# idra-lab/safe-mpc

Hardware: AMD Instinct MI355X
Metric: RTI-MPC instance-steps/s (batch=4096 per GPU, Z1 N=30) (higher is better)
Workload: dtype f64; 1 GPU; C1: Z1-class 6-DoF, N=30, 4096 instances/GPU, controller st (soft terminal NN row, MLP 12-256-256-256-1 fp32), EXT cost exact Hessian, 6 capsule pairs, Halton x0; batch_per_gpu=4096, batch_total=4096, horizon=30, controller=st, streams_per_gpu=3, qp_form=throughput, hip_graphs=False

## Files before the change

safe_mpc_amd/csrc/engine.hip:

```cpp
#include <hip/hip_runtime.h>

#include <cstdarg>
#include <cstdio>
#include <cstring>
#include <new>
#include <type_traits>
#include <vector>

#include "../../include/smpc.h"
#include "kernel_qp.hpp"
#include "kernel_qp_wg.hpp"
#include "kernel_build.hpp"
#include "kernels_callers.hpp"
#include "kernels_policy.hpp"
#include "kernels_mlp.hpp"
#include "kernels_nodes.hpp"
#include "kernels_sqp.hpp"
#include "kernels_guess.hpp"
#include "kernels_score.hpp"
#include "kernels_ik.hpp"
#include "kernels_rays.hpp"
#include "kernels_forecast.hpp"

using namespace smpc;
// ... 250 lines not shown
        if (!d) return nullptr;
        if (up && e == hipSuccess) e = hipMemcpyAsync(d, host, sizeof(T) * n, hipMemcpyHostToDevice, h->stream);
        if (down && host) back.push_back({(void*)host, d, sizeof(T) * n});
        return d;
    }
    template <class T> const T* in(const T* host, size_t n) { return view(host, n, true, false); }
    template <class T> T* out(T* host, size_t n) { return view(host, n, false, true); }
    template <class T> T* inout(T* host, size_t n) { return view(host, n, true, true); }

    template <class F> int place(F&& views) {
        views(*this);
        if (dev) return SMPC_OK;
        int rc;
        if ((rc = h->d_stage.reserve(h, "staging buffer", c.off))) return rc;
        c = Carve{h->d_stage.p};
        views(*this);
        if (e != hipSuccess) return fail(h, SMPC_EHIP, "staging copy failed: %s", hipGetErrorString(e));
        return SMPC_OK;
    }
    int finish() {
        if (dev) return SMPC_OK;
        for (const Back& b : back) HIPCHK(h, hipMemcpyAsync(b.host, b.dev, b.bytes, hipMemcpyDeviceToHost, h->stream));
        HIPCHK(h, hipStreamSynchronize(h->stream));
        return SMPC_OK;
    }
};

size_t ws_doubles_per_instance(smpc_handle* h, int N) {
    size_t per = 0;
    with_nq(h, [&](auto NQ) { per = QpLayout<NQ>(h->desc.n_rows).per_instance(N); return SMPC_OK; });
    return per;
}

int upload_bounds(smpc_handle* h, const double* lo, const double* hi) {
    const int nx = 2 * h->desc.nq;
    std::vector<double> l((size_t)(h->N + 1) * nx), u((size_t)(h->N + 1) * nx);
    for (int k = 0; k <= h->N; k++)
        for (int i = 0; i < nx; i++) {
            l[(size_t)k * nx + i] = lo ? lo[(size_t)k * nx + i] : (k == h->N ? h->desc.x_lo_e[i] : h->desc.x_lo[i]);
            u[(size_t)k * nx + i] = hi ? hi[(size_t)k * nx + i] : (k == h->N ? h->desc.x_hi_e[i] : h->desc.x_hi[i]);
        }
    int rc;
    if ((rc = h->d_lo.reserve(h, "stage bounds", l.size() * sizeof(double))) ||
        (rc = h->d_hi.reserve(h, "stage bounds", u.size() * sizeof(double))))
        return rc;
    HIPCHK(h, hipMemcpyAsync(h->d_lo.p, l.data(), l.size() * sizeof(double), hipMemcpyHostToDevice, h->stream));
    HIPCHK(h, hipMemcpyAsync(h->d_hi.p, u.data(), u.size() * sizeof(double), hipMemcpyHostToDevice, h->stream));
    HIPCHK(h, hipStreamSynchronize(h->stream));
    return SMPC_OK;
}

int ensure_mlp(smpc_handle* h, size_t M, int level = 2) {
    const size_t Mp = (M + 127) / 128 * 128, row = sizeof(float) * Mp, H = h->net->H;
    int rc;
    if ((rc = h->d_y.reserve(h, "network output", row))) return rc;
    for (int l = 0; level >= 1 && l + 1 < h->net->nlayers; l++)
        if ((rc = h->d_dg[l].reserve(h, "network activation derivatives", row * H))) return rc;
    if (level < 2) return SMPC_OK;
    if ((rc = h->d_S.reserve(h, "network features", row * MLP_KPAD)) || (rc = h->d_GS.reserve(h, "network gradients", row * MLP_NPAD)) ||
        (rc = h->d_dA.reserve(h, "network backward pass", row * H)) || (rc = h->d_dB.reserve(h, "network backward pass", row * H)))
        return rc;
    for (int l = 0; l + 1 < h->net->nlayers; l++)
        if ((rc = h->d_act[l].reserve(h, "network activations", row * H))) return rc;
    return SMPC_OK;
}

// ... 205 lines not shown
        return f > 0.0 && f <= 1.0 ? f : QP_CREW_DEFAULT;
    }();
    return v;
}
static int qp_crew_waves(const smpc_handle* h, int B) {
    const int pairs = (B + 1) / 2;
    if (h->qp_crew_waves > 0) return h->qp_crew_waves < pairs ? h->qp_crew_waves : pairs;
    const double f = h->qp_crew > 0.0 ? h->qp_crew : qp_crew_default();
    const int g = (int)ceil(f * pairs);
    return g < 1 ? 1 : (g > pairs ? pairs : g);
}

template <class F> int with_rows(const smpc_handle* h, F&& f) {
    switch (h->desc.n_rows) {
    case 6: return f(std::integral_constant<int, 6>{});
    case 4: return f(std::integral_constant<int, 4>{});
    default: return f(std::integral_constant<int, -1>{});
    }
}

int ensure_instance_bounds(smpc_handle* h, int B, bool zero) { return h->bounds.room(h, (size_t)2 * B * (h->N + 1) * 2 * h->desc.nq, zero); }
double* instance_hi(const smpc_handle* h) { return h->bounds.d.p ? h->bounds.d.p + h->bounds.d.cap / (2 * sizeof(double)) : nullptr; }

struct StageBounds {
    const double *lo, *hi;
    long stride;
};
StageBounds stage_bounds(const smpc_handle* h, int B) {
    if (const double* lo = h->bounds.for_batch(B)) return {lo, instance_hi(h), (long)(h->N + 1) * 2 * h->desc.nq};
    return {h->d_lo.p, h->d_hi.p, 0L};
}

template <int NQ>
int launch_stage_records(smpc_handle* h, int B, const double* x0, const double* xg, const double* ug, const double* p, bool timed) {
    int rc;
    if ((rc = launch_nn<NQ>(h, B, xg, p, h->d_nn.p, h->desc.nn_mode == SMPC_NN_TERMINAL ? 2 : 1))) return rc;
    if (timed) HIPCHK(h, hipEventRecord(h->ev_t[1], h->stream));
    const StageBounds bd = stage_bounds(h, B);
    const long nodes = (long)B * (h->N + 1);
    const dim3 grd((unsigned)((nodes + 64 / SB_G - 1) / (64 / SB_G))), blk(64);
    const double* nn = h->desc.nn_mode != SMPC_NN_NONE ? h->d_nn.p : nullptr;
    int32_t* const zero_cnt = h->desc.nn_mode == SMPC_NN_ALL ? h->d_nn_cnt : nullptr;
    with_rows(h, [&](auto MR) {
        return with_scene(h, B, [&](auto SCENE, auto sc) {
            return with_model(h, B, [&](auto MODEL, auto... md) {
                return with_row_bounds(h, B, [&](auto... rb) {
                    hipLaunchKernelGGL((k_stage_build<NQ, MR, SCENE, MODEL>), grd, blk, 0, h->stream, h->d_desc, B, h->N, x0, xg, ug, p, bd.lo,
                                       bd.hi, h->d_zl.p, nn, h->d_ws.p, bd.stride, h->d_active, zero_cnt, sc, md..., rb...);
                    return SMPC_OK;
                });
            });
        });
    });
    HIPCHK(h, hipGetLastError());
    if (timed) { HIPCHK(h, hipEventRecord(h->ev_t[2], h->stream)); HIPCHK(h, hipEventRecord(h->ev_t[4], h->stream)); }
    return SMPC_OK;
}

template <int NQ>
int launch_stage_records_per_node(smpc_handle* h, int B, const double* x0, const double* xg, const double* ug, const double* p) {
    int rc;
    if ((rc = launch_eval<NQ>(h, B, xg, ug, p, h->d_ev.p))) return rc;
    const StageBounds bd = stage_bounds(h, B);
    const int tiles = (int)ev_tiles((size_t)B * (h->N + 1));
    with_rows(h, [&](auto MR) {
        return with_row_bounds(h, B, [&](auto... rb) {
            hipLaunchKernelGGL((k_qp_setup<NQ, MR>), dim3(tiles), dim3(32 * EV_TILE), 0, h->stream, h->d_desc, B, h->N, x0, xg, ug, p, bd.lo,
                               bd.hi, h->d_zl.p, h->d_ev.p, h->d_ws.p, bd.stride, h->d_active, rb...);
            return SMPC_OK;
        });
    });
    HIPCHK(h, hipGetLastError());
    return SMPC_OK;
}

#ifndef QP_WG_FULL_BATCH
#define QP_WG_FULL_BATCH 256
#endif
#ifndef QP_WG_MAX_BATCH
#define QP_WG_MAX_BATCH 1024
#endif
static int qp_wg_mode() {
    static const int v = [] { const char* e = getenv("SMPC_QP_WG"); return e ? atoi(e) : -1; }();
    return v;
}
static int qp_wg_max_batch() {
    static const int v = [] { const char* e = getenv("SMPC_QP_WG_MAX_BATCH"); return e ? atoi(e) : QP_WG_MAX_BATCH; }();
    return v;
}
static int qp_wg_full_batch() {
    static const int v = [] { const char* e = getenv("SMPC_QP_WG_FULL_BATCH"); return e ? atoi(e) : QP_WG_FULL_BATCH; }();
    return v;
}
constexpr size_t QP_WG_LDS_LIMIT = 160 * 1024 - 512;

template <int NQ> int qp_wg_choice(const smpc_handle* h, int B) {
    const int mode = h->qp_mode >= -1 ? h->qp_mode : qp_wg_mode();
    if (mode == 0) return 0;
    if (mode < 0 && B > qp_wg_max_batch()) return 0;
    const auto fits = [&](int nhw) { return (size_t)WgLds<NQ>(h->N, h->desc.n_rows, nhw).total * sizeof(double) <= QP_WG_LDS_LIMIT; };
    if (B <= qp_wg_full_batch() && fits(8)) return 8;
    return fits(4) ? 4 : 0;
}

template <int NQ, int NHW>
int launch_qp_wg(smpc_handle* h, int B, const double* x0, const double* xg, const double* ug, double* xo, double* uo, int32_t* st,
                 int32_t* it) {
    if (h->d_hrec.cap < sizeof(double) * B * (h->N + 1) * HRecLayout<NQ>::SIZE)
        return fail(h, SMPC_ESTATE, "latency-form records not grown for %d instances", B);
    const size_t lds = (size_t)WgLds<NQ>(h->N, h->desc.n_rows, NHW).total * sizeof(double);
    return with_rows(h, [&](auto MR) {
        hipLaunchKernelGGL((k_qp_ipm_wg<NQ, MR, NHW>), dim3(B), dim3(32 * NHW), lds, h->stream, h->d_desc, B, h->N, x0, xg, ug, h->d_ws.p,
                           h->d_hrec.p, xo, uo, st, it, h->d_last_it.p, h->d_active, h->d_ord_hist.p);
        return SMPC_OK;
    });
}

template <int NQ, int NHW> int raise_qp_wg_lds_limit(smpc_handle* h) {
    if (h->wg_lds_raised[NHW == 8 ? 0 : 1]) return SMPC_OK;
    const int rc = with_rows(h, [&](auto MR) {
        HIPCHK(h, hipFuncSetAttribute(reinterpret_cast<const void*>(&k_qp_ipm_wg<NQ, MR, NHW>), hipFuncAttributeMaxDynamicSharedMemorySize,
                                      (int)QP_WG_LDS_LIMIT));
        return SMPC_OK;
    });
    h->wg_lds_raised[NHW == 8 ? 0 : 1] = rc == SMPC_OK;
    return rc;
}

template <int NQ> int ensure_qp_wg(smpc_handle* h, int B) {
    const int nhw = qp_wg_choice<NQ>(h, B);
    if (nhw == 0) return SMPC_OK;
    int rc;
    if ((rc = h->d_hrec.reserve(h, "latency-form records", sizeof(double) * B * (h->N + 1) * HRecLayout<NQ>::SIZE))) return rc;
    return nhw == 8 ? raise_qp_wg_lds_limit<NQ, 8>(h) : raise_qp_wg_lds_limit<NQ, 4>(h);
}

template <int NQ>
int launch_solve(smpc_handle* h, int B, const double* x0, const double* xg, const double* ug, const double* p,
                 double* xo, double* uo, int32_t* st, int32_t* it) {
    int rc;
    h->timing_now = false;
    if (h->timing) {
        h->timing_now = !capturing(h);
    }
    const bool timed = h->timing_now;
    if (timed) {
        h->ev_cur = (h->ev_cur + 1) % smpc_handle::EV_RING;
        h->ev_t = h->ev_sets[h->ev_cur];
        h->ev_complete[h->ev_cur] = false;
        h->timed_count++;
        HIPCHK(h, hipEventRecord(h->ev_t[0], h->stream));
    }
    if ((rc = launch_stage_records<NQ>(h, B, x0, xg, ug, p, timed))) return rc;
    const int wg_nhw = qp_wg_choice<NQ>(h, B);
    const bool wg = wg_nhw > 0;
    const int32_t* order = nullptr;
    if (h->order_B == B && B > 1 && !wg) {
        hipLaunchKernelGGL(k_order_by_iters, dim3((B + ORD_PER_BLOCK - 1) / ORD_PER_BLOCK), dim3(64), 0, h->stream, B, h->d_last_it.p,
                           h->d_order.p, h->d_ord_hist.p, h->d_ord_hist.p + 256, h->d_ord_hist.p + 512);
        order = h->d_order.p;
    } else {
        HIPCHK(h, hipMemsetAsync(h->d_ord_hist.p, 0, 520 * sizeof(int32_t), h->stream));
    }
    unsigned long long* wstat = nullptr;
    if (timed && h->timing == 1) {
        const unsigned long long init[4] = {0ull, ~0ull, 0ull, 0ull};
        HIPCHK(h, hipMemcpyAsync(h->d_wstat.p, init, sizeof(init), hipMemcpyHostToDevice, h->stream));
        wstat = h->d_wstat.p;
    }
    if (wg) {
        if ((rc = wg_nhw == 8 ? launch_qp_wg<NQ, 8>(h, B, x0, xg, ug, xo, uo, st, it) : launch_qp_wg<NQ, 4>(h, B, x0, xg, ug, xo, uo, st, it))) return rc;
    } else {
        const bool nt = qp_nt_mode() < 0 ? ws_doubles_per_instance(h, h->N) * sizeof(double) * (size_t)B >= qp_nt_threshold : qp_nt_mode() > 0;
        with_rows(h, [&](auto MR) {
            const auto launch = [&](auto NT) {
                hipLaunchKernelGGL((k_qp_ipm<NQ, MR, NT>), dim3(qp_crew_form<NQ, MR>() ? qp_crew_waves(h, B) : (B + 1) / 2), dim3(64), 0, h->stream, h->d_desc, B, h->N, x0, xg, ug,
                                   h->d_ws.p, xo, uo, st, it, order, h->d_last_it.p, wstat, h->d_active, h->d_ord_hist.p, h->d_ord_hist.p + 513);
                return SMPC_OK;
            };
            if constexpr (MR < 0) return launch(std::false_type{});
            else return nt ? launch(std::true_type{}) : launch(std::false_type{});
        });
    }
    h->order_B = B;
    HIPCHK(h, hipGetLastError());
    if (timed) {
        HIPCHK(h, hipEventRecord(h->ev_t[3], h->stream));
        h->ev_complete[h->ev_cur] = true;
        h->timed = 1;
    }
    return SMPC_OK;
}

struct ChkBlock { double *x_min, *x_max, *row_lb, *row_ub; size_t doubles; };
ChkBlock chk_block(double* base, int nq) {
    Carve m = dense(base);
    ChkBlock b{};
    b.x_min = m.take<double>(2 * nq);
    b.x_max = m.take<double>(2 * nq);
    b.row_lb = m.take<double>(SMPC_MAX_ROWS);
    b.row_ub = m.take<double>(SMPC_MAX_ROWS);
    b.doubles = m.off / sizeof(double);
    return b;
}
int upload_check_bounds(smpc_handle* h, const double* x_min, const double* x_max, const double* row_lb_chk,
                        const double* row_ub_chk) {
    const int nq = h->desc.nq, nr = h->desc.n_rows;
    std::vector<double> img(chk_block(nullptr, nq).doubles, 0.0);
    const ChkBlock b = chk_block(img.data(), nq);
    put(b.x_min, x_min, 2 * nq);
// ... 204 lines not shown
        h->d_active = nullptr;
        if (rc) { h->mlp_rows_hint = 0; return rc; }
        h->mlp_rows_hint = rows_test;
        hipLaunchKernelGGL(k_par_safe_list, grid(S * (N + 1)), blk, 0, s, (int)S, N, K, stepping, c.list, c.n_open, st->r, c.st,
                           h->d_nn_idx.p, h->d_nn_cnt);
        const ChkBlock cb = chk_block(h->chk.d.p, nq);
        const long M = S * (N + 1);
        rc = with_nq(h, [&](auto NQ) {
            hipLaunchKernelGGL((k_par_check_state<NQ>), grid(M), blk, 0, s, h->d_desc, (int)S, N, c.n_open, c.xo, cb.x_min, cb.x_max, par->tol_x,
                               cb.row_lb, cb.row_ub, c.st, c.ok, coll);
            HIPCHK(h, hipGetLastError());
            if (const int e = run_mlp<NQ>(h, (int)M, 3, 0, c.xo, false, rows_of_nodes(N + 1))) return e;
            hipLaunchKernelGGL((k_check_nn<NQ>), grid(M), blk, 0, s, h->d_desc, (int)M, c.xo, par->alpha, par->tol_safe, h->d_y.p, c.safe,
                               h->d_nn_idx.p, h->d_nn_cnt);
            HIPCHK(h, hipGetLastError());
            return SMPC_OK;
        });
        if (rc) { h->mlp_rows_hint = 0; return rc; }
    }
    h->mlp_rows_hint = 0;
    hipLaunchKernelGGL(k_par_select, grid(B), blk, 0, s, B, N, nq, stepping, d_ok, d_safe, c.pos, c.st, c.it, c.ok, c.safe, c.xo, c.uo,
                       st->x_temp, st->u_temp, st->status, st->qp_iter, st->x_guess, st->fails, st->current_step, st->r, st->x_viable,
                       d_acc, d_act, abort_out, any_abort, h->d_nn_cnt);
    hipLaunchKernelGGL(k_provide_control, grid((long)B * (nx + nq)), blk, 0, s, B, N, nq, d_acc, st->x_temp, st->u_temp, st->x_guess,
                       st->u_guess, u_out, stepping, d_act, u_other);
    HIPCHK(h, hipGetLastError());
    return SMPC_OK;
}

int ensure_batch(smpc_handle* h, int B, bool with_ev) {
    const size_t nodes = (size_t)B * (h->N + 1);
    const size_t nn_nodes = h->desc.nn_mode == SMPC_NN_NONE ? 0 : (h->desc.nn_mode == SMPC_NN_TERMINAL ? (size_t)B : nodes);
    int rc;
    if ((with_ev && (rc = h->d_ev.reserve(h, "linearisation records", sizeof(double) * ev_tiles(nodes) * EV_TILE * EV_D))) ||
        (rc = h->d_ws.reserve(h, "QP workspace", sizeof(double) * ws_doubles_per_instance(h, h->N) * B)) ||
        (rc = h->d_nn.reserve(h, "network rows", sizeof(double) * nn_nodes * (1 + 2 * h->desc.nq), true)) ||
        (rc = h->d_order.reserve(h, "dispatch order", sizeof(int32_t) * B)))
        return rc;
    const size_t had = h->d_last_it.cap;
    rc = h->d_last_it.reserve(h, "iteration counts", sizeof(int32_t) * B);
    if (h->d_last_it.cap != had) h->order_B = 0;
    if (rc || (rc = h->d_ord_hist.reserve(h, "iteration histogram", sizeof(int32_t) * 520, true))) return rc;
    return with_nq(h, [&](auto NQ) { return ensure_qp_wg<NQ>(h, B); });
}

struct SqpScratch {
    double *xs, *us, *dx, *du, *xt, *step, *m0t, *mt, *alpha, *m0, *Dd;
    int32_t *st, *it, *pos, *n_open;
    uint8_t *act, *settled, *trial;
    size_t bytes;
};
SqpScratch sqp_layout(char* base, int B, int N, int nq, bool full) {
    const size_t nX = (size_t)B * (N + 1) * 2 * nq, nU = (size_t)B * N * nq;
    Carve m{base};
    SqpScratch w{};
    w.xt = m.take<double>(nX);
    w.pos = m.take<int32_t>((size_t)B * (N + 1));
    if (full) {
        w.xs = m.take<double>(nX);
        w.us = m.take<double>(nU);
        w.dx = m.take<double>(nX);
        w.du = m.take<double>(nU);
        w.step = m.take<double>(B);
        w.m0t = m.take<double>((size_t)3 * B);
        w.mt = m.take<double>((size_t)3 * B);
        w.alpha = m.take<double>(B);
        w.m0 = m.take<double>(B);
        w.Dd = m.take<double>(B);
// ... 1586 lines not shown
        if (nc > ctx_cap) return fail(h, SMPC_EINVAL, "smpc_debug_scene_slots: the context holds %zu floats, room for %zu", nc, ctx_cap);
        HIPCHK(h, hipMemcpy(ctx_out, h->ctx.d.p, nc * sizeof(float), hipMemcpyDeviceToHost));
    }
    return SMPC_OK;
}

extern "C" int smpc_debug_qp_dispatch(smpc_handle* h, int32_t* out) {
    if (!h || !out) return SMPC_EINVAL;
    (void)hipSetDevice(h->device);
    if (!h->d_ord_hist.p) return fail(h, SMPC_ESTATE, "smpc_debug_qp_dispatch: no solve yet");
    HIPCHK(h, hipStreamSynchronize(h->stream));
    HIPCHK(h, hipMemcpy(out, h->d_ord_hist.p, 520 * sizeof(int32_t), hipMemcpyDeviceToHost));
    return SMPC_OK;
}

extern "C" int smpc_debug_stage_records(smpc_handle* h, int B, const double* x0, const double* xg, const double* ug, const double* p,
                                        int path, double* ws_out, int32_t* layout) {
    if (!h || B <= 0 || !x0 || !xg || !ug || !p || !ws_out || !layout) return SMPC_EINVAL;
    (void)hipSetDevice(h->device);
    int rc;
    if ((rc = guard_solve_slots(h, B, "smpc_debug_stage_records"))) return rc;
    if ((rc = ensure_batch(h, B))) return rc;
    const int N = h->N, nx = 2 * h->desc.nq, nu = h->desc.nq;
    Stage io{h, false};
    const double *dx0, *dxg, *dug, *dp;
    if ((rc = io.place([&](Stage& v) {
             dx0 = v.in(x0, (size_t)B * nx);
             dxg = v.in(xg, (size_t)B * (N + 1) * nx);
             dug = v.in(ug, (size_t)B * N * nu);
             dp = v.in(p, (size_t)B * (N + 1) * SMPC_NP);
         })))
        return rc;
    const size_t per = ws_doubles_per_instance(h, N);
    HIPCHK(h, hipMemsetAsync(h->d_ws.p, 0, per * (size_t)B * sizeof(double), h->stream));
    (void)&launch_stage_records<5>, (void)&launch_stage_records_per_node<5>;
    (void)&launch_stage_records<6>, (void)&launch_stage_records_per_node<6>;
    (void)&launch_stage_records<7>, (void)&launch_stage_records_per_node<7>;
    if ((rc = with_nq(h, [&](auto NQ) {
             return path == 1 ? launch_stage_records<NQ>(h, B, dx0, dxg, dug, dp, false) : launch_stage_records_per_node<NQ>(h, B, dx0, dxg, dug, dp);
         })))
        return rc;
    HIPCHK(h, hipMemcpyAsync(ws_out, h->d_ws.p, per * (size_t)B * sizeof(double), hipMemcpyDeviceToHost, h->stream));
    if ((rc = io.finish())) return rc;
    return with_nq(h, [&](auto NQ) {
        const QpLayout<NQ> Ly(h->desc.n_rows);
        const int v[24] = {Ly.stride, Ly.nIMG, Ly.oIMG, Ly.oSL, Ly.nF, Ly.oR0, Ly.oR1, Ly.oR2, Ly.oCZA, Ly.oCZN, Ly.oZ, Ly.oZN, Ly.NRT, Ly.nJ,
                           (int)per, 12, Ly.iTT, Ly.iGT, Ly.iGN, Ly.iB, Ly.iSC, Ly.iHQQ, Ly.iGZ, 0};
        for (int i = 0; i < 24; i++) layout[i] = v[i];
        return SMPC_OK;
    });
}

#ifdef QP_PROFILE
extern "C" int smpc_debug_qp_profile(unsigned long long* out16) {
    unsigned long long zero[16] = {0};
    if (hipMemcpyFromSymbol(out16, HIP_SYMBOL(smpc::g_qp_prof), sizeof(zero)) != hipSuccess) return -1;
    if (hipMemcpyToSymbol(HIP_SYMBOL(smpc::g_qp_prof), zero, sizeof(zero)) != hipSuccess) return -1;
    return 0;
}
extern "C" int smpc_debug_qp_wg_profile(unsigned long long* out16) {
    unsigned long long zero[16] = {0};
    if (hipMemcpyFromSymbol(out16, HIP_SYMBOL(smpc::g_wg_prof), sizeof(zero)) != hipSuccess) return -1;
    if (hipMemcpyToSymbol(HIP_SYMBOL(smpc::g_wg_prof), zero, sizeof(zero)) != hipSuccess) return -1;
    return 0;
}
#endif
```

safe_mpc_amd/csrc/kernel_build.hpp:

```cpp
#pragma once
#include "kernel_qp.hpp"
#include "rnea_deriv.hpp"

namespace smpc {

constexpr int SB_G = 8;
#ifndef SB_WAVES
#define SB_WAVES 2
#endif

template <int NQ, int MR_MAX> struct SbLds {
    static constexpr int NX = 2 * NQ;
    static constexpr int X_SC = 0, XA_END = 2 * NQ;
    static constexpr int X_SPC = 0, SPC_D = 24, XR_END = SPC_D * NQ;
    static constexpr int X_PT = 0, X_ZP = X_PT + 3 * SMPC_MAX_POINTS, XG_END = X_ZP + 9 * NQ;
    static constexpr int X_E = 0, X_Z0 = NX, X_GQ = X_Z0 + NX, XS_END = X_GQ + NQ;
    static constexpr int m1 = XA_END > XR_END ? XA_END : XR_END, m2 = XG_END > XS_END ? XG_END : XS_END;
    static constexpr int SIZE = qp_even_c(m1 > m2 ? m1 : m2);
};

template <int OFF> __device__ __forceinline__ double dpp_up(double x) {
    static_assert(OFF >= 1 && OFF <= 15, "row_shl:1..15");
    int lo = __double2loint(x), hi = __double2hiint(x);
    lo = __builtin_amdgcn_update_dpp(0, lo, 0x100 + OFF, 0xf, 0xf, true);
    hi = __builtin_amdgcn_update_dpp(0, hi, 0x100 + OFF, 0xf, 0xf, true);
    return __hiloint2double(hi, lo);
}

template <int CTRL> __device__ __forceinline__ double dpp_mov(double x) {
    int lo = __double2loint(x), hi = __double2hiint(x);
    lo = __builtin_amdgcn_update_dpp(0, lo, CTRL, 0xf, 0xf, true);
    hi = __builtin_amdgcn_update_dpp(0, hi, CTRL, 0xf, 0xf, true);
    return __hiloint2double(hi, lo);
}
__device__ __forceinline__ double grp_sum(double v) {
    v += dpp_mov<0xB1>(v);
    v += dpp_mov<0x4E>(v);
    v += dpp_mov<0x141>(v);
    return v;
}
__device__ __forceinline__ double grp_max(double v) {
    v = fmax(v, dpp_mov<0xB1>(v));
    v = fmax(v, dpp_mov<0x4E>(v));
    v = fmax(v, dpp_mov<0x141>(v));
    return v;
}

template <int NQ, int MRT, bool SCENE = false, bool MODEL = false, bool ROWB = false>
__device__ __forceinline__ void stage_build(const smpc_problem_desc* __restrict__ D, const QpLayout<NQ>& Ly, const int N, const int k,
                                            const bool valid, const int g, double* __restrict__ L, const double* __restrict__ x0b,
                                            const double* __restrict__ xk, const double* __restrict__ uk, const double* __restrict__ pk,
                                            const double* __restrict__ lo_k, const double* __restrict__ hi_k,
                                            const double* __restrict__ zl_st, const double* __restrict__ nnk, double* __restrict__ w,
                                            const double* __restrict__ geom_b = nullptr, const smpc_joint* __restrict__ Jb = nullptr,
                                            const double* __restrict__ rb_k = nullptr, const size_t rb_half = 0) {
    constexpr int NX = 2 * NQ, NU = NQ, NZ = 3 * NQ, NQP = QpLayout<NQ>::NQP, NZP = QpLayout<NQ>::NZP;
    constexpr int MR_MAX = MRT >= 0 ? MRT : SMPC_MAX_ROWS;
    constexpr int NSLOT = (MR_MAX + SB_G - 1) / SB_G;
    constexpr int NNL = SB_G - 1;
    static_assert(NQ < SB_G, "lane SB_G - 1 carries the network's row, lanes 0 .. NQ - 1 a joint each");
    static_assert(MR_MAX <= 2 * SB_G && 2 * NQ <= 2 * SB_G, "at most two collision rows and two box rows per lane");
    using LD = SbLds<NQ, MR_MAX>;
    const int MR = Ly.MR, MRP = Ly.MRP;
    const int rT0 = NX, rC0 = NX + NQ, rNN = NX + NQ + MR;
    const bool last = (k == N);
    const bool jl = g < NQ;
    const int gj = jl ? g : NQ - 1;
    double* const sX = L;
    const double dt = D->dt, cB = 0.5 * dt * dt;

    double qd[NQ], qdd[NQ];
#pragma unroll
    for (int i = 0; i < NQ; i++) {
        qd[i] = xk[NQ + i];
        qdd[i] = last ? 0.0 : uk[i];
    }
    {
        double s, c;
        sincos(xk[gj], &s, &c);
        if (jl) { sX[LD::X_SC + 2 * g] = s; sX[LD::X_SC + 2 * g + 1] = c; }
    }
    lds_fence();

// ... 308 lines not shown
    }
    double* const sE = sX + LD::X_E;
    double* const sZ0 = sX + LD::X_Z0;
    double* const sGQ = sX + LD::X_GQ;
    for (int i = g; i < NX; i += SB_G) sZ0[i] = k == 0 ? x0b[i] - xk[i] : 0.0;
    if (jl) sGQ[g] = gz_q;
    lds_fence();
    double bmax = 0.0;
    auto defect = [&](int i) -> double {
        if (last) return 0.0;
        const double* xn = xk + NX;
        const int ii = i < NQ ? i : i - NQ;
        const double ukk = uk[ii];
        return i < NQ ? xk[ii] + dt * xk[NQ + ii] + cB * ukk - xn[ii] : xk[NQ + ii] + dt * ukk - xn[NQ + ii];
    };
    for (int i = g; i < NX; i += SB_G) {
        const double bb = defect(i);
        bmax = fmax(bmax, fabs(bb));
        if (valid) *(w + Ly.oIMG + Ly.iB + i) = bb;
    }
    bmax = grp_max(bmax);
    const double bflag = bmax > 0.0 ? 1.0 : 0.0;
    auto gz_u = [&](int c) -> double { return (reach && !last) ? cs * 2.0 * D->R * uk[c] : 0.0; };
    for (int hz = g; hz < NZP; hz += SB_G) {
        if (hz >= NU && hz < NU + NQ) continue;
        if (valid) *(w + Ly.oIMG + Ly.iGZ + hz) = hz < NU ? gz_u(hz) : 0.0;
    }
    if (jl && valid) *(w + Ly.oIMG + Ly.iGZ + NU + g) = gz_q;
    if (g < 4 && valid) {
        const double huu = (reach && !last ? cs * 2.0 * D->R : 0.0) + lm;
        *(w + Ly.oIMG + Ly.iSC + g) = g == 0 ? huu : (g == 1 ? lm : (g == 2 ? wsoft : bflag));
        *(w + Ly.oSL + g) = g == 0 ? wsoft : (g == 1 ? bflag : 0.0);
    }
    if (valid) *(w + Ly.oWC + g) = 0.0;

    double r0_loc = 0.0, mu_acc = 0.0, inf0 = 0.0;
    int cnt = 0;
    auto init_row = [&](bool present, int r, double lo, double hi, double cz, double cn, bool soft) -> double {
        double tl = 1.0, ll = 0.0, tu = 1.0, lu = 0.0;
        if (present) {
            const double thr = soft ? QP_THR : QP_THR_HARD * (cn > 0.0 ? cn : 1.0);
            if (lo > -QP_ABSENT) {
                const double s0 = soft ? QP_THR : 0.0;
                const double slack = cz + s0 - lo;
                tl = fmax(slack, thr);
                ll = D->qp_mu0 / tl;
                if (soft) ll = fmin(ll, 0.5 * wsoft);
                r0_loc = fmax(r0_loc, fabs(slack - tl));
                cnt += soft ? 2 : 1;
                mu_acc += ll * tl;
                if (soft) { mu_acc += (wsoft - ll) * s0; tu = s0; }
            }
            if (hi < QP_ABSENT) {
                const double slack = hi - cz;
                tu = fmax(slack, thr);
                lu = D->qp_mu0 / tu;
                r0_loc = fmax(r0_loc, fabs(slack - tu));
                cnt += 1;
                mu_acc += lu * tu;
            }
            if (valid) {
                reinterpret_cast<dbl2*>(w + Ly.oR0)[r] = dbl2{lo, hi};
                reinterpret_cast<dbl2*>(w + Ly.oR1)[r] = dbl2{tl, tu};
                reinterpret_cast<dbl2*>(w + Ly.oR2)[r] = dbl2{ll, lu};
            }
        }
        return -(ll - lu);
// ... 35 lines not shown
        } else {
            if (k >= 1 && fabs(row.lb) < SMPC_INF) lo = row.lb - growv[sl];
            if (k >= 1 && fabs(row.ub) < SMPC_INF) hi = row.ub - growv[sl];
        }
#pragma unroll
        for (int j = 0; j < NQ; j++) cn = fmax(cn, fabs(grow[sl][j]));
        if (k == 0) {
#pragma unroll
            for (int j = 0; j < NQ; j++) cz = fma(grow[sl][j], sZ0[j], cz);
        }
        eC[sl] = init_row(have, rC0 + r, lo, hi, cz, cn, false);
        if (!have) eC[sl] = 0.0;
        if (have && k == 0 && D->rows_at_node0) {
            const double v = growv[sl] + cz;
            if constexpr (ROWB) {
                if ((fabs(lb) < SMPC_INF && v < lb - D->qp_tol) || (fabs(ub) < SMPC_INF && v > ub + D->qp_tol)) inf0 = 1.0;
            } else {
                if ((fabs(row.lb) < SMPC_INF && v < row.lb - D->qp_tol) || (fabs(row.ub) < SMPC_INF && v > row.ub + D->qp_tol)) inf0 = 1.0;
            }
        }
    }
    double eN = 0.0;
    {
        const bool mine = g == NNL;
        double lo = -QP_ABSENT, cn = 0.0;
        if (nn_on && mine) {
            lo = 0.0 - nnk[0];
            for (int i = 0; i < NX; i++) cn = fmax(cn, fabs(nnk[1 + i]));
        }
        eN = init_row(mine, rNN, lo, QP_ABSENT, 0.0, cn, wsoft >= 0.0);
        if (!mine) eN = 0.0;
    }
    for (int r = g; r < 32; r += SB_G)
        if (valid) { *(w + Ly.oCZA + r) = 0.0; *(w + Ly.oCZN + r) = 0.0; }
    for (int hz = g; hz < NZ; hz += SB_G) {
        const double z0 = hz >= NU ? sZ0[hz - NU] : 0.0;
        if (valid) { *(w + Ly.oZ + hz) = z0; *(w + Ly.oZN + hz) = z0; }
    }
    lds_fence();
    {
        double pc[NZ];
#pragma unroll
        for (int c = 0; c < NZ; c++) pc[c] = rowT[c] * eT;
#pragma unroll
        for (int sl = 0; sl < NSLOT; sl++)
#pragma unroll
            for (int j = 0; j < NQ; j++) pc[NU + j] = fma(grow[sl][j], eC[sl], pc[NU + j]);
        if (nn_on && g == NNL) {
#pragma unroll
            for (int i = 0; i < NX; i++) pc[NU + i] = fma(nnk[1 + i], eN, pc[NU + i]);
        }
#pragma unroll
        for (int c = 0; c < NZ; c++) {
            const double sc = grp_sum(pc[c]);
            const bool skip = (k == 0 && c >= NU) || (last && c < NU);
            const double gz = c < NU ? gz_u(c) : (c < NU + NQ ? sGQ[c - NU] : 0.0);
            const double a = gz + sc + (c >= NU ? sE[c - NU] : 0.0);
            r0_loc = fmax(r0_loc, skip ? 0.0 : fabs(a));
        }
    }
    if (!last) {
        for (int i = g; i < NX; i += SB_G) {
            double ax = 0.0;
            if (k == 0) ax = i < NQ ? sZ0[i] + dt * sZ0[NQ + i] : sZ0[i];
            r0_loc = fmax(r0_loc, fabs(ax + defect(i)));
        }
    }
    const double R0 = grp_max(r0_loc), musum = grp_sum(mu_acc), cntsum = grp_sum((double)cnt), infs = grp_max(inf0);
    if (g < 4 && valid) w[Ly.oPART + g] = g == 0 ? R0 : (g == 1 ? musum : (g == 2 ? cntsum : infs));

    if (valid) {
        double* img = w + Ly.oIMG;
        if (g < NQP) {
#pragma unroll
            for (int c = 0; c < NZ; c++) *(img + Ly.iTT + c * NQP + g) = rowT[c];
        }
#pragma unroll
        for (int sl = 0; sl < NSLOT; sl++) {
            const int r = g + SB_G * sl;
            if (r < MRP) {
#pragma unroll
                for (int j = 0; j < NQ; j++) *(img + Ly.iGT + j * MRP + r) = grow[sl][j];
            }
        }
        if (g == NNL)
            for (int i = 0; i < NX; i++) *(img + Ly.iGN + i) = nn_on ? nnk[1 + i] : 0.0;
    }
    lds_fence();
}

template <int NQ, int MRT, bool SCENE = false, bool MODEL = false, class... MJ>
__global__ __launch_bounds__(64) __attribute__((amdgpu_waves_per_eu(SB_WAVES, SB_WAVES))) void k_stage_build(const smpc_problem_desc* __restrict__ D, int B, int N, const double* __restrict__ x0,
                                                    const double* __restrict__ xg, const double* __restrict__ ug, const double* __restrict__ pp,
                                                    const double* __restrict__ lo_st, const double* __restrict__ hi_st,
                                                    const double* __restrict__ zl_st, const double* __restrict__ nn, double* __restrict__ ws_all,
                                                    long bnd_stride, const uint8_t* __restrict__ active, int32_t* __restrict__ zero_cnt,
                                                    const SceneArg<SCENE> sc = {}, const MJ* __restrict__... md) {
    static_assert(ModelRowArg<MODEL, MJ...>, "md: the table of smpc_joint records when MODEL is set, then the row-bounds table or nothing");
    constexpr bool ROWB = RowBounds<MJ...>;
    constexpr int NX = 2 * NQ, NU = NQ;
    constexpr int MR_MAX = MRT >= 0 ? MRT : SMPC_MAX_ROWS;
    using LD = SbLds<NQ, MR_MAX>;
    if (zero_cnt && blockIdx.x == 0 && threadIdx.x == 0) *zero_cnt = 0;
    constexpr int NODES = 64 / SB_G;
    __shared__ __attribute__((aligned(16))) double smem[NODES * LD::SIZE];
    const int g = threadIdx.x & (SB_G - 1), grp = threadIdx.x / SB_G;
    const long total = (long)B * (N + 1);
    long t = (long)blockIdx.x * NODES + grp;
    bool valid = t < total;
    if (!valid) t = total - 1;
    const long b = t / (N + 1);
    const int k = (int)(t - b * (N + 1));
    if (active && !active[b]) valid = false;
    const QpLayout<NQ> Ly(MRT >= 0 ? MRT : D->n_rows);
    double* w = ws_all + (size_t)b * Ly.per_instance(N) + (size_t)k * Ly.stride;
    const double* xk = xg + ((size_t)b * (N + 1) + k) * NX;
    const double* uk = ug + ((size_t)b * N + (k < N ? k : N - 1)) * NU;
    const double* pk = pp + ((size_t)b * (N + 1) + k) * SMPC_NP;
    const size_t bo = (size_t)b * bnd_stride + (size_t)k * NX;
    const double* geom_b = nullptr;
    if constexpr (SCENE) geom_b = scene_block(sc, b, scene_time(sc) + k, Ly.MR);
    const smpc_joint* Jb = nullptr;
    if constexpr (MODEL) Jb = model_joints<NQ>(D, b, md...);
    const double* rb_k = nullptr;
    size_t rb_half = 0;
    if constexpr (ROWB) {
        rb_k = row_bounds_table(md...) + ((size_t)b * (N + 1) + k) * Ly.MR;
        rb_half = (size_t)B * (N + 1) * Ly.MR;
    }
    stage_build<NQ, MRT, SCENE, MODEL, ROWB>(D, Ly, N, k, valid, g, smem + grp * LD::SIZE, x0 + (size_t)b * NX, xk, uk, pk, lo_st + bo, hi_st + bo, zl_st,
                                nn ? nn + (D->nn_mode == SMPC_NN_TERMINAL ? (size_t)b : (size_t)b * (N + 1) + k) * (1 + NX) : nullptr, w,
                                geom_b, Jb, rb_k, rb_half);
}

}
```

safe_mpc_amd/csrc/kernel_qp.hpp:

```cpp
#pragma once
#include <type_traits>

#include "device_model.hpp"

namespace smpc {

constexpr double QP_THR = 1e-1;
constexpr double QP_THR_HARD = 3e-2;
constexpr double QP_FTB = 0.995;
constexpr double QP_ALPHA_MIN = 1e-12;
constexpr double QP_ABSENT = 1e300;

constexpr int qp_even_c(int n) { return (n + 1) & ~1; }
constexpr int qp_al8(int n) { return (n + 7) & ~7; }

template <int NQ> struct QpLayout {
    static constexpr int NX = 2 * NQ, NU = NQ, NZ = 3 * NQ;
    static constexpr int NZP = qp_even_c(NZ), NQP = qp_even_c(NQ), WS2 = qp_even_c(NX + 1);
    static constexpr int LC0 = WS2;
    static constexpr int KS = qp_even_c(LC0 + NQ);
    static constexpr int WR = NX + 1, LOFF = NQ * WR, NWP = qp_even_c(LOFF + NQ * (NQ + 1) / 2);
    __host__ __device__ static constexpr int w_coff(int j) { return LOFF + j * NQ - j * (j - 1) / 2; }
    int MR, MRP, NRC, NRT;
    int iTT, iGT, iGN, iHQQ, iGZ, iB, iSC, nIMG;
    int nJ;
    int nF;
    int oIMG, oW, oSL, oPART, oWC, oR0, oR1, oR2, oCZA, oCZN;
    int oZ, oZN, oA12;
    int stride;
    __host__ __device__ explicit QpLayout(int n_rows) {
        MR = n_rows;
        MRP = qp_even_c(MR);
        NRC = NQ + MR + 1;
        NRT = NX + NRC;
        int i = 0;
        iTT = i; i += NZ * NQP;
        iGT = i; i += NQ * MRP;
        iGN = i; i += NX;
        nJ = i;
        iB = i; i += NX;
        iSC = i; i += 4;
        nF = i;
        iHQQ = i; i += qp_even_c(NQ * NQ);
        iGZ = i; i += NZP;
        nIMG = i;
        int o = 0;
        oIMG = o; o += qp_al8(nIMG);
        oW = o; o += qp_al8(NWP);
        oSL = o; o += 16;
        oPART = oSL + 4;
        oWC = oSL + 8;
        oR0 = o; o += qp_al8(NRT * 2);
        oR1 = o; o += qp_al8(NRT * 2);
        oR2 = o; o += qp_al8(NRT * 2);
        oCZA = o; o += 32;
        oCZN = o; o += 32;
        oZ = o; o += qp_al8(NZ);
        oZN = o; o += qp_al8(NZ);
        oA12 = o; o += qp_al8(2 * NZ);
        static_assert(NQ <= 8, "the corrector's w shares a 16-double block with the stage scalars");
        stride = (o + 15) & ~15;
    }
    __host__ __device__ size_t per_instance(int N) const { return (size_t)stride * (N + 1); }
};

typedef double dbl2 __attribute__((ext_vector_type(2)));


__device__ __forceinline__ void lds_fence() {
    __builtin_amdgcn_fence(__ATOMIC_ACQ_REL, "wavefront", "local");
    __builtin_amdgcn_wave_barrier();
}

__device__ __forceinline__ void hold(double& a, double& b, double& c, double& d) { asm volatile("" : "+v"(a), "+v"(b), "+v"(c), "+v"(d)); }
template <int H> __device__ __forceinline__ void hold_rows2(dbl2 (&a)[H], dbl2 (&b)[H], double (&s)[5]) {
    static_assert(H == 3 || H == 4, "NQP / 2 of the built sizes");
    if constexpr (H == 3)
        asm volatile("" : "+v"(a[0]), "+v"(a[1]), "+v"(a[2]), "+v"(b[0]), "+v"(b[1]), "+v"(b[2]), "+v"(s[0]), "+v"(s[1]), "+v"(s[2]),
                          "+v"(s[3]), "+v"(s[4]));
    else
        asm volatile("" : "+v"(a[0]), "+v"(a[1]), "+v"(a[2]), "+v"(a[3]), "+v"(b[0]), "+v"(b[1]), "+v"(b[2]), "+v"(b[3]), "+v"(s[0]),
                          "+v"(s[1]), "+v"(s[2]), "+v"(s[3]), "+v"(s[4]));
}
template <int H> __device__ __forceinline__ void hold_rows4(dbl2 (&a)[H], dbl2 (&b)[H], dbl2 (&c)[H], dbl2 (&d)[H], double (&s)[9]) {
    static_assert(H == 3 || H == 4, "NQP / 2 of the built sizes");
    if constexpr (H == 3)
        asm volatile("" : "+v"(a[0]), "+v"(a[1]), "+v"(a[2]), "+v"(b[0]), "+v"(b[1]), "+v"(b[2]), "+v"(c[0]), "+v"(c[1]), "+v"(c[2]),
// ... 302 lines not shown
                cn = 0.0;
                for (int c = 0; c < NZ; c++) {
                    const double cv = sC[(r - NX) * NZP + c];
                    cz = fma(cv, sZ0[c], cz);
                    cn = fmax(cn, fabs(cv));
                }
            }
            const bool soft = (r == rNN) && wsoft >= 0.0;
            const double thr = soft ? QP_THR : QP_THR_HARD * (cn > 0.0 ? cn : 1.0);
            if (sLO[r] > -QP_ABSENT) {
                const double s0 = soft ? QP_THR : 0.0;
                const double slack = cz + s0 - sLO[r];
                tl = fmax(slack, thr);
                ll = D->qp_mu0 / tl;
                if (soft) ll = fmin(ll, 0.5 * wsoft);
                r0_loc = fmax(r0_loc, fabs(slack - tl));
                cnt += soft ? 2 : 1;
                mu_acc += ll * tl;
                if (soft) { mu_acc += (wsoft - ll) * s0; tu = s0; }
            }
            if (sHI[r] < QP_ABSENT) {
                const double slack = sHI[r] - cz;
                tu = fmax(slack, thr);
                lu = D->qp_mu0 / tu;
                r0_loc = fmax(r0_loc, fabs(slack - tu));
                cnt += 1;
                mu_acc += lu * tu;
            }
        }
        if (r < NRT) {
            reinterpret_cast<dbl2*>(w + Ly.oR1)[r] = dbl2{tl, tu};
            reinterpret_cast<dbl2*>(w + Ly.oR2)[r] = dbl2{ll, lu};
        }
        *(w + Ly.oCZA + hl) = 0.0;
        *(w + Ly.oCZN + hl) = 0.0;
        sE[r] = -(ll - lu);
    }
    if (hl < 4) *(w + Ly.oSL + hl) = hl == 0 ? wsoft : (hl == 1 ? bflag : 0.0);
    if (hl < 8) *(w + Ly.oWC + hl) = 0.0;
    if (hl < NZ) { *(w + Ly.oZ + hl) = sZ0[hl]; *(w + Ly.oZN + hl) = sZ0[hl]; }
    lds_fence();
    if (hl < NZ && !(k == 0 && hl >= NU) && !(last && hl < NU)) {
        double a = sGZ[hl];
        for (int r = 0; r < NRC; r++) a = fma(sC[r * NZP + hl], sE[NX + r], a);
        if (hl >= NU) a += sE[hl - NU];
        r0_loc = fmax(r0_loc, fabs(a));
    }
    if (!last && hl < NX) {
        double ax = 0.0;
        if (k == 0) ax = hl < NQ ? sZ0[NU + hl] + dt * sZ0[NU + NQ + hl] : sZ0[NU + hl];
        r0_loc = fmax(r0_loc, fabs(ax + sB[hl]));
    }
    double inf0 = 0.0;
    if (k == 0 && D->rows_at_node0 && hl >= rC0 && hl < rNN) {
        const smpc_row& row = D->rows[hl - rC0];
        double v = e.row_val[hl - rC0];
        for (int c = 0; c < NZ; c++) v = fma(sC[(hl - NX) * NZP + c], sZ0[c], v);
        if constexpr (RowBounds<RB...>) {
            const RowLbUb own = row_bounds_at(row_bounds_table(rb...), B, N, MR, b, k, hl - rC0);
            if ((fabs(own.lb) < SMPC_INF && v < own.lb - D->qp_tol) || (fabs(own.ub) < SMPC_INF && v > own.ub + D->qp_tol)) inf0 = 1.0;
        } else {
            if ((fabs(row.lb) < SMPC_INF && v < row.lb - D->qp_tol) || (fabs(row.ub) < SMPC_INF && v > row.ub + D->qp_tol)) inf0 = 1.0;
        }
    }
    const double R0 = half_max(r0_loc), musum = half_sum(mu_acc), cntsum = half_sum((double)cnt), infs = half_max(inf0);
    if (hl < 4) w[Ly.oPART + hl] = hl == 0 ? R0 : (hl == 1 ? musum : (hl == 2 ? cntsum : infs));
}

#ifndef QP_WAVES_PER_EU
#define QP_WAVES_PER_EU 2
#endif

template <int NQ, int MRT> constexpr bool qp_crew_form() { return !(NQ == 6 && MRT < 0); }
// ... 230 lines not shown
    const double inv_m = 1.0 / (double)m_comp;
    QPT(13);

    double rho_lin = 1.0, alpha = 0.0, sigmu = 0.0, corr_w = 1.0;
    bool pending = false;
    int it = 0, st_code = 2;
    const double tol = D->qp_tol;
    const double tol_r = D->qp_tol_res > 0.0 ? D->qp_tol_res : D->qp_tol;
    const int max_iter = D->qp_max_iter;
    const int stall_max = D->qp_stall_iters;
    int stall = 0;
    bool broke = false;
    double *Pc = sIMG + O_PA, *Pn = sIMG + O_PB2;
    double *pvc = sIMG + O_PVA, *pvn = sIMG + O_PVB;
    lds_fence();

    for (it = 0; it < max_iter; it++) {
        if (mu <= tol && rho_lin * R0 <= tol_r) { st_code = 0; break; }

        double mu_new = 0.0;
        {
            dbl2 img[IMG_PF];
            QpRow rs;
            dbl2 slb;
            double zc, znc, czar, cznr;
            auto load_b1 = [&](int k) {
                const double* w = stage_ptr(k);
                const dbl2* s2 = reinterpret_cast<const dbl2*>(w + Ly.oIMG);
#pragma unroll
                for (int j = 0; j < IMG_PF; j++) img[j] = ldnt(s2 + min(hl + 32 * j, img_n2 - 1));
                const dbl2 r0 = ldnt(reinterpret_cast<const dbl2*>(w + Ly.oR0) + hr), r1 = ldnt(reinterpret_cast<const dbl2*>(w + Ly.oR1) + hr),
                           r2 = ldnt(reinterpret_cast<const dbl2*>(w + Ly.oR2) + hr);
                rs.lo = r0.x; rs.hi = r0.y; rs.tl = r1.x; rs.tu = r1.y; rs.ll = r2.x; rs.lu = r2.y;
                czar = *(w + Ly.oCZA + hr);
                cznr = *(w + Ly.oCZN + hr);
                slb = *reinterpret_cast<const dbl2*>(w + Ly.oSL);
                zc = *(w + Ly.oZ + hz);
                znc = *(w + Ly.oZN + hz);
            };
            auto stage_b1 = [&](int k, auto last_tag) {
                constexpr bool last = decltype(last_tag)::value;
                asm volatile("; QPMARK B1_BEGIN");
                double* w = stage_ptr(k);
                {
                    dbl2* d2 = reinterpret_cast<dbl2*>(sIMG);
#pragma unroll
                    for (int j = 0; j < IMG_PF; j++) d2[min(hl + 32 * j, img_n2 - 1)] = img[j];
                }
                const double wsoft = slb.x;
                const bool bflag = !last && slb.y != 0.0;
                {
                    const bool soft = soft_lane && wsoft >= 0.0;
                    double rr_ = 0.0, s1_ = 0.0, s2_ = 0.0;
                    const QpDir rd = qp_row_dir<false>(rs, soft, wsoft, cznr, sigmu, corr_w, czar, &rr_, &s1_, &s2_, nullptr, nullptr);
                    rs.tl += alpha * rd.dtl; rs.ll += alpha * rd.dll;
                    rs.tu += alpha * rd.dtu; rs.lu += alpha * rd.dlu;
                    stnt_b1(dbl2{rs.tl, rs.tu}, reinterpret_cast<dbl2*>(w + Ly.oR1) + hr);
                    stnt_b1(dbl2{rs.ll, rs.lu}, reinterpret_cast<dbl2*>(w + Ly.oR2) + hr);
                    double Dr;
                    sE[hr] = qp_row_coeff(rs, soft, wsoft, 0.0, 0.0, 0.0, &Dr);
                    sD[hr] = Dr;
                    mu_new += row_live ? qp_row_comp(rs, soft, wsoft) : 0.0;
                }
                zc += alpha * (znc - zc);
                *(w + Ly.oZ + hz) = zc;
                lds_fence();
                QPT(0);
                load_b1(k > 0 ? k - 1 : 0);
                {
                    double a = bflag ? pdot(Pc + hl_x * NX, sB, NX / 2) : 0.0;
                    if constexpr (last && PASS_TAB) asm volatile("" : "+v"(a));
// ... 622 lines not shown
        __builtin_amdgcn_fence(__ATOMIC_RELEASE, "workgroup");

        double rr_max, S1c, S2c;
        sweep_f(std::true_type{}, &rr_max, &S1c, &S2c);
        __builtin_amdgcn_fence(__ATOMIC_RELEASE, "workgroup");
        const double a_max = rr_max > 0.0 ? 1.0 / rr_max : 1e300;
        const double tau_k = a_max >= 0.99 ? fmin(0.9999, fmax(QP_FTB, 1.0 - mu)) : QP_FTB;
        alpha = fmin(1.0, tau_k * a_max);
        if (!(alpha == alpha)) { st_code = 4; break; }
        if (alpha < QP_ALPHA_MIN) { st_code = 3; break; }
        pending = true;
        rho_lin *= (1.0 - alpha);
        const double mu_before = mu;
        mu = (mu * (double)m_comp + alpha * S1c + alpha * alpha * S2c) * inv_m;
        if (!(mu == mu)) { st_code = 4; pending = false; break; }
        {
            const bool stalled = alpha < 0.5 && !(mu < 0.5 * mu_before);
            stall = stalled ? stall + 0x10001 : (stall & ~0xffff);
        }
        if (stall_max > 0 && ((stall & 0xffff) >= stall_max || (stall >> 16) >= stall_max + (stall_max + 5) / 6) &&
            !(mu <= tol && rho_lin * R0 <= tol_r)) { st_code = 5; it++; break; }
    }
    if (it == max_iter && st_code == 2 && mu <= tol && rho_lin * R0 <= tol_r) st_code = 0;

    bool bad = false;
    const double a_fin = pending ? alpha : 0.0;
    constexpr int EP_CH = 8;
    for (int k0 = 0; k0 <= N; k0 += EP_CH) {
        double zz[EP_CH], zzn[EP_CH], bb[EP_CH];
#pragma unroll
        for (int j = 0; j < EP_CH; j++) {
            const int k = k0 + j <= N ? k0 + j : N;
            const double* w = ws + (size_t)k * Ly.stride;
            zz[j] = *(w + Ly.oZ + hz);
            zzn[j] = *(w + Ly.oZN + hz);
            const int ku = k < N ? k : N - 1;
            bb[j] = hl < NU ? ub0[(size_t)ku * NU + hl_u] : xb0[(size_t)k * NX + hl_px];
        }
#pragma unroll
        for (int j = 0; j < EP_CH; j++) {
            const int k = k0 + j;
            const double v = pending ? bb[j] + zz[j] + a_fin * (zzn[j] - zz[j]) : bb[j] + zz[j];
            if (k <= N) {
                if (hl < NU) {
                    if (k < N) { u_out[((size_t)b * N + k) * NU + hl] = v; bad |= !(v == v); }
                } else if (hl < NZ) {
                    x_out[((size_t)b * (N + 1) + k) * NX + hl - NU] = v;
                    bad |= !(v == v);
                }
            }
        }
    }
    const bool any_bad = half_max(bad ? 1.0 : 0.0) > 0.0;
#ifdef QP_PROFILE
    QPT(12);
    if (hl == 0) {
        for (int i = 0; i < 14; i++) atomicAdd(&g_qp_prof[i], tacc[i]);
        atomicAdd(&g_qp_prof[14], 1ull);
        atomicAdd(&g_qp_prof[15], (unsigned long long)it);
    }
#endif
    if (wstat && hl == 0) {
        const unsigned long long t_end = __builtin_amdgcn_s_memrealtime(), t_begin = s_tbegin[half];
        atomicAdd(&wstat[0], t_end - t_begin);
        atomicMin(&wstat[1], t_begin);
        atomicMax(&wstat[2], t_end);
        atomicAdd(&wstat[3], 1ull);
// ... 66 lines not shown
```

Measured before the change: 1.147 million instance-steps/s.

## Skip per-stage zeroing of iterate slots via shared zero header in workspace

Adds a zeroed header block ahead of the QP workspace. On the first IPM iteration, stages k>0 read their initial CZA/CZN/Z values from that shared header instead of their own slots, so the stage-build and setup kernels no longer write zeros and initial iterates for every stage (only k==0, or all stages when the workgroup solver is used). It also reorders the R0/R1/R2 row records into one contiguous block. The aim is fewer global stores during setup. The risk is correctness: ws_all minus stride must land on the header, and stage-local initial values for the primal part are replaced by the header's zeros for k>0.

```diff
diff --git a/safe_mpc_amd/csrc/engine.hip b/safe_mpc_amd/csrc/engine.hip
--- a/safe_mpc_amd/csrc/engine.hip
+++ b/safe_mpc_amd/csrc/engine.hip
@@ -306,6 +306,9 @@
     return per;
 }
 
+size_t ws_header_doubles(smpc_handle* h) { return ws_doubles_per_instance(h, 0); }
+double* qp_ws(smpc_handle* h) { return h->d_ws.p + ws_header_doubles(h); }
+
 int upload_bounds(smpc_handle* h, const double* lo, const double* hi) {
     const int nx = 2 * h->desc.nq;
     std::vector<double> l((size_t)(h->N + 1) * nx), u((size_t)(h->N + 1) * nx);
@@ -577,7 +580,8 @@
 }
 
 template <int NQ>
-int launch_stage_records(smpc_handle* h, int B, const double* x0, const double* xg, const double* ug, const double* p, bool timed) {
+int launch_stage_records(smpc_handle* h, int B, const double* x0, const double* xg, const double* ug, const double* p, bool timed,
+                         bool all_starts) {
     int rc;
     if ((rc = launch_nn<NQ>(h, B, xg, p, h->d_nn.p, h->desc.nn_mode == SMPC_NN_TERMINAL ? 2 : 1))) return rc;
     if (timed) HIPCHK(h, hipEventRecord(h->ev_t[1], h->stream));
@@ -591,7 +595,7 @@
             return with_model(h, B, [&](auto MODEL, auto... md) {
                 return with_row_bounds(h, B, [&](auto... rb) {
                     hipLaunchKernelGGL((k_stage_build<NQ, MR, SCENE, MODEL>), grd, blk, 0, h->stream, h->d_desc, B, h->N, x0, xg, ug, p, bd.lo,
-                                       bd.hi, h->d_zl.p, nn, h->d_ws.p, bd.stride, h->d_active, zero_cnt, sc, md..., rb...);
+                                       bd.hi, h->d_zl.p, nn, qp_ws(h), bd.stride, h->d_active, zero_cnt, all_starts ? 1 : 0, sc, md..., rb...);
                     return SMPC_OK;
                 });
             });
@@ -611,7 +615,7 @@
     with_rows(h, [&](auto MR) {
         return with_row_bounds(h, B, [&](auto... rb) {
             hipLaunchKernelGGL((k_qp_setup<NQ, MR>), dim3(tiles), dim3(32 * EV_TILE), 0, h->stream, h->d_desc, B, h->N, x0, xg, ug, p, bd.lo,
-                               bd.hi, h->d_zl.p, h->d_ev.p, h->d_ws.p, bd.stride, h->d_active, rb...);
+                               bd.hi, h->d_zl.p, h->d_ev.p, qp_ws(h), bd.stride, h->d_active, rb...);
             return SMPC_OK;
         });
     });
@@ -655,7 +659,7 @@
         return fail(h, SMPC_ESTATE, "latency-form records not grown for %d instances", B);
     const size_t lds = (size_t)WgLds<NQ>(h->N, h->desc.n_rows, NHW).total * sizeof(double);
     return with_rows(h, [&](auto MR) {
-        hipLaunchKernelGGL((k_qp_ipm_wg<NQ, MR, NHW>), dim3(B), dim3(32 * NHW), lds, h->stream, h->d_desc, B, h->N, x0, xg, ug, h->d_ws.p,
+        hipLaunchKernelGGL((k_qp_ipm_wg<NQ, MR, NHW>), dim3(B), dim3(32 * NHW), lds, h->stream, h->d_desc, B, h->N, x0, xg, ug, qp_ws(h),
                            h->d_hrec.p, xo, uo, st, it, h->d_last_it.p, h->d_active, h->d_ord_hist.p);
         return SMPC_OK;
     });
@@ -696,9 +700,9 @@
         h->timed_count++;
         HIPCHK(h, hipEventRecord(h->ev_t[0], h->stream));
     }
-    if ((rc = launch_stage_records<NQ>(h, B, x0, xg, ug, p, timed))) return rc;
     const int wg_nhw = qp_wg_choice<NQ>(h, B);
     const bool wg = wg_nhw > 0;
+    if ((rc = launch_stage_records<NQ>(h, B, x0, xg, ug, p, timed, wg))) return rc;
     const int32_t* order = nullptr;
     if (h->order_B == B && B > 1 && !wg) {
         hipLaunchKernelGGL(k_order_by_iters, dim3((B + ORD_PER_BLOCK - 1) / ORD_PER_BLOCK), dim3(64), 0, h->stream, B, h->d_last_it.p,
@@ -720,7 +724,7 @@
         with_rows(h, [&](auto MR) {
             const auto launch = [&](auto NT) {
                 hipLaunchKernelGGL((k_qp_ipm<NQ, MR, NT>), dim3(qp_crew_form<NQ, MR>() ? qp_crew_waves(h, B) : (B + 1) / 2), dim3(64), 0, h->stream, h->d_desc, B, h->N, x0, xg, ug,
-                                   h->d_ws.p, xo, uo, st, it, order, h->d_last_it.p, wstat, h->d_active, h->d_ord_hist.p, h->d_ord_hist.p + 513);
+                                   qp_ws(h), xo, uo, st, it, order, h->d_last_it.p, wstat, h->d_active, h->d_ord_hist.p, h->d_ord_hist.p + 513);
                 return SMPC_OK;
             };
             if constexpr (MR < 0) return launch(std::false_type{});
@@ -991,8 +995,10 @@
     const size_t nodes = (size_t)B * (h->N + 1);
     const size_t nn_nodes = h->desc.nn_mode == SMPC_NN_NONE ? 0 : (h->desc.nn_mode == SMPC_NN_TERMINAL ? (size_t)B : nodes);
     int rc;
+    const size_t ws_had = h->d_ws.cap;
+    if ((rc = h->d_ws.reserve(h, "QP workspace", sizeof(double) * (ws_header_doubles(h) + ws_doubles_per_instance(h, h->N) * B)))) return rc;
+    if (h->d_ws.cap != ws_had) HIPCHK(h, hipMemsetAsync(h->d_ws.p, 0, sizeof(double) * ws_header_doubles(h), h->stream));
     if ((with_ev && (rc = h->d_ev.reserve(h, "linearisation records", sizeof(double) * ev_tiles(nodes) * EV_TILE * EV_D))) ||
-        (rc = h->d_ws.reserve(h, "QP workspace", sizeof(double) * ws_doubles_per_instance(h, h->N) * B)) ||
         (rc = h->d_nn.reserve(h, "network rows", sizeof(double) * nn_nodes * (1 + 2 * h->desc.nq), true)) ||
         (rc = h->d_order.reserve(h, "dispatch order", sizeof(int32_t) * B)))
         return rc;
@@ -2645,15 +2651,15 @@
          })))
         return rc;
     const size_t per = ws_doubles_per_instance(h, N);
-    HIPCHK(h, hipMemsetAsync(h->d_ws.p, 0, per * (size_t)B * sizeof(double), h->stream));
+    HIPCHK(h, hipMemsetAsync(qp_ws(h), 0, per * (size_t)B * sizeof(double), h->stream));
     (void)&launch_stage_records<5>, (void)&launch_stage_records_per_node<5>;
     (void)&launch_stage_records<6>, (void)&launch_stage_records_per_node<6>;
     (void)&launch_stage_records<7>, (void)&launch_stage_records_per_node<7>;
     if ((rc = with_nq(h, [&](auto NQ) {
-             return path == 1 ? launch_stage_records<NQ>(h, B, dx0, dxg, dug, dp, false) : launch_stage_records_per_node<NQ>(h, B, dx0, dxg, dug, dp);
+             return path == 1 ? launch_stage_records<NQ>(h, B, dx0, dxg, dug, dp, false, false) : launch_stage_records_per_node<NQ>(h, B, dx0, dxg, dug, dp);
          })))
         return rc;
-    HIPCHK(h, hipMemcpyAsync(ws_out, h->d_ws.p, per * (size_t)B * sizeof(double), hipMemcpyDeviceToHost, h->stream));
+    HIPCHK(h, hipMemcpyAsync(ws_out, qp_ws(h), per * (size_t)B * sizeof(double), hipMemcpyDeviceToHost, h->stream));
     if ((rc = io.finish())) return rc;
     return with_nq(h, [&](auto NQ) {
         const QpLayout<NQ> Ly(h->desc.n_rows);
diff --git a/safe_mpc_amd/csrc/kernel_build.hpp b/safe_mpc_amd/csrc/kernel_build.hpp
--- a/safe_mpc_amd/csrc/kernel_build.hpp
+++ b/safe_mpc_amd/csrc/kernel_build.hpp
@@ -48,7 +48,7 @@
 
 template <int NQ, int MRT, bool SCENE = false, bool MODEL = false, bool ROWB = false>
 __device__ __forceinline__ void stage_build(const smpc_problem_desc* __restrict__ D, const QpLayout<NQ>& Ly, const int N, const int k,
-                                            const bool valid, const int g, double* __restrict__ L, const double* __restrict__ x0b,
+                                            const bool valid, const bool starts, const int g, double* __restrict__ L, const double* __restrict__ x0b,
                                             const double* __restrict__ xk, const double* __restrict__ uk, const double* __restrict__ pk,
                                             const double* __restrict__ lo_k, const double* __restrict__ hi_k,
                                             const double* __restrict__ zl_st, const double* __restrict__ nnk, double* __restrict__ w,
@@ -423,7 +423,6 @@
         *(w + Ly.oIMG + Ly.iSC + g) = g == 0 ? huu : (g == 1 ? lm : (g == 2 ? wsoft : bflag));
         *(w + Ly.oSL + g) = g == 0 ? wsoft : (g == 1 ? bflag : 0.0);
     }
-    if (valid) *(w + Ly.oWC + g) = 0.0;
 
     double r0_loc = 0.0, mu_acc = 0.0, inf0 = 0.0;
     int cnt = 0;
@@ -525,10 +524,10 @@
         if (!mine) eN = 0.0;
     }
     for (int r = g; r < 32; r += SB_G)
-        if (valid) { *(w + Ly.oCZA + r) = 0.0; *(w + Ly.oCZN + r) = 0.0; }
+        if (valid && starts) { *(w + Ly.oCZA + r) = 0.0; *(w + Ly.oCZN + r) = 0.0; }
     for (int hz = g; hz < NZ; hz += SB_G) {
         const double z0 = hz >= NU ? sZ0[hz - NU] : 0.0;
-        if (valid) { *(w + Ly.oZ + hz) = z0; *(w + Ly.oZN + hz) = z0; }
+        if (valid && starts) { *(w + Ly.oZ + hz) = z0; *(w + Ly.oZN + hz) = z0; }
     }
     lds_fence();
     {
@@ -588,7 +587,7 @@
                                                     const double* __restrict__ lo_st, const double* __restrict__ hi_st,
                                                     const double* __restrict__ zl_st, const double* __restrict__ nn, double* __restrict__ ws_all,
                                                     long bnd_stride, const uint8_t* __restrict__ active, int32_t* __restrict__ zero_cnt,
-                                                    const SceneArg<SCENE> sc = {}, const MJ* __restrict__... md) {
+                                                    int all_starts, const SceneArg<SCENE> sc = {}, const MJ* __restrict__... md) {
     static_assert(ModelRowArg<MODEL, MJ...>, "md: the table of smpc_joint records when MODEL is set, then the row-bounds table or nothing");
     constexpr bool ROWB = RowBounds<MJ...>;
     constexpr int NX = 2 * NQ, NU = NQ;
@@ -621,7 +620,7 @@
         rb_k = row_bounds_table(md...) + ((size_t)b * (N + 1) + k) * Ly.MR;
         rb_half = (size_t)B * (N + 1) * Ly.MR;
     }
-    stage_build<NQ, MRT, SCENE, MODEL, ROWB>(D, Ly, N, k, valid, g, smem + grp * LD::SIZE, x0 + (size_t)b * NX, xk, uk, pk, lo_st + bo, hi_st + bo, zl_st,
+    stage_build<NQ, MRT, SCENE, MODEL, ROWB>(D, Ly, N, k, valid, k == 0 || all_starts != 0, g, smem + grp * LD::SIZE, x0 + (size_t)b * NX, xk, uk, pk, lo_st + bo, hi_st + bo, zl_st,
                                 nn ? nn + (D->nn_mode == SMPC_NN_TERMINAL ? (size_t)b : (size_t)b * (N + 1) + k) * (1 + NX) : nullptr, w,
                                 geom_b, Jb, rb_k, rb_half);
 }
diff --git a/safe_mpc_amd/csrc/kernel_qp.hpp b/safe_mpc_amd/csrc/kernel_qp.hpp
--- a/safe_mpc_amd/csrc/kernel_qp.hpp
+++ b/safe_mpc_amd/csrc/kernel_qp.hpp
@@ -50,9 +50,10 @@
         oSL = o; o += 16;
         oPART = oSL + 4;
         oWC = oSL + 8;
-        oR0 = o; o += qp_al8(NRT * 2);
-        oR1 = o; o += qp_al8(NRT * 2);
-        oR2 = o; o += qp_al8(NRT * 2);
+        oR1 = o;
+        oR2 = oR1 + NRT * 2;
+        oR0 = oR2 + NRT * 2;
+        o += qp_al8(NRT * 6);
         oCZA = o; o += 32;
         oCZN = o; o += 32;
         oZ = o; o += qp_al8(NZ);
@@ -421,13 +422,14 @@
             reinterpret_cast<dbl2*>(w + Ly.oR1)[r] = dbl2{tl, tu};
             reinterpret_cast<dbl2*>(w + Ly.oR2)[r] = dbl2{ll, lu};
         }
-        *(w + Ly.oCZA + hl) = 0.0;
-        *(w + Ly.oCZN + hl) = 0.0;
+        if (k == 0) {
+            *(w + Ly.oCZA + hl) = 0.0;
+            *(w + Ly.oCZN + hl) = 0.0;
+        }
         sE[r] = -(ll - lu);
     }
     if (hl < 4) *(w + Ly.oSL + hl) = hl == 0 ? wsoft : (hl == 1 ? bflag : 0.0);
-    if (hl < 8) *(w + Ly.oWC + hl) = 0.0;
-    if (hl < NZ) { *(w + Ly.oZ + hl) = sZ0[hl]; *(w + Ly.oZN + hl) = sZ0[hl]; }
+    if (k == 0 && hl < NZ) { *(w + Ly.oZ + hl) = sZ0[hl]; *(w + Ly.oZN + hl) = sZ0[hl]; }
     lds_fence();
     if (hl < NZ && !(k == 0 && hl >= NU) && !(last && hl < NU)) {
         double a = sGZ[hl];
@@ -724,11 +726,12 @@
                 const dbl2 r0 = ldnt(reinterpret_cast<const dbl2*>(w + Ly.oR0) + hr), r1 = ldnt(reinterpret_cast<const dbl2*>(w + Ly.oR1) + hr),
                            r2 = ldnt(reinterpret_cast<const dbl2*>(w + Ly.oR2) + hr);
                 rs.lo = r0.x; rs.hi = r0.y; rs.tl = r1.x; rs.tu = r1.y; rs.ll = r2.x; rs.lu = r2.y;
-                czar = *(w + Ly.oCZA + hr);
-                cznr = *(w + Ly.oCZN + hr);
+                const double* ws0 = (it == 0 && k > 0) ? ws_all - Ly.stride : w;
+                czar = *(ws0 + Ly.oCZA + hr);
+                cznr = *(ws0 + Ly.oCZN + hr);
                 slb = *reinterpret_cast<const dbl2*>(w + Ly.oSL);
-                zc = *(w + Ly.oZ + hz);
-                znc = *(w + Ly.oZN + hz);
+                zc = *(ws0 + Ly.oZ + hz);
+                znc = *(ws0 + Ly.oZN + hz);
             };
             auto stage_b1 = [&](int k, auto last_tag) {
                 constexpr bool last = decltype(last_tag)::value;
@@ -1417,7 +1420,7 @@
         for (int j = 0; j < EP_CH; j++) {
             const int k = k0 + j <= N ? k0 + j : N;
             const double* w = ws + (size_t)k * Ly.stride;
-            zz[j] = *(w + Ly.oZ + hz);
+            zz[j] = *((it == 0 && k > 0 ? ws_all - Ly.stride : w) + Ly.oZ + hz);
             zzn[j] = *(w + Ly.oZN + hz);
             const int ku = k < N ? k : N - 1;
             bb[j] = hl < NU ? ub0[(size_t)ku * NU + hl_u] : xb0[(size_t)k * NX + hl_px];
```

Result: no change. 1.145 million instance-steps/s (-0.1%).
